# romanoshiliarhopoulos/Backgammon-Engine

Hardware: NVIDIA B200
Metric: selfplay_plies_per_sec (higher is better)
Workload: dtype f32

## Files before the change

### backgammon-engine_b200/csrc/bgx_kernels.cuh

```cuda
#pragma once
#include "bgx_device.cuh"
#include "bgx_ply.cuh"

namespace bgx {

constexpr int kGameWarps = 16;
constexpr int kGameThreads = kGameWarps * 32;
struct WarpSeat {
    long long slot;
    unsigned long long gid;
    int ply, step, status, player;
    int carry;
    int dice_base;
};

template <int kWarps, int kSets>
constexpr int ply_smem()
{
    return kFixedBytes + kWarps * (int)sizeof(PlyScratch<kSets>) + (int)sizeof(StealShared<kWarps>) + kWarps * (int)sizeof(WarpSeat) + 16;
}

template <int W, int S>
struct PlyConfig {
    static constexpr int kWarps = W, kSets = S, kSmem = ply_smem<W, S>();
// ... 7 lines not shown
    {
        int rc = 0;
        ((rc = rc ? rc : f(C{})), ...);
        return rc;
    }
    template <typename F>
    static void dispatch(int warps, F &&f) { ((warps == C::kWarps ? f(C{}) : void()), ...); }
};
using PlyConfigs = PlyConfigList<PlyConfig<16, 109>, PlyConfig<20, 86>, PlyConfig<24, 72>, PlyConfig<32, 53>>;
constexpr int kEvalSmem = kFixedBytes + 16;

constexpr int kUniqSlots = 4096;
constexpr int kUniqWords = 8;
constexpr size_t kUniqBytesPerWarp = (size_t)kUniqSlots * kUniqWords * 4;

__global__ void k_build_table(const float *__restrict__ flat, float *__restrict__ Wt)
{
    const int idx = blockIdx.x * blockDim.x + threadIdx.x;
    if (idx >= kTableFloats) return;
    const int f = idx / kHidden, j = idx % kHidden;
    Wt[idx] = flat[j * kFeatures + f];
}

__global__ void k_fixed_scale(const float *__restrict__ flat, float *__restrict__ aux)
{
    __shared__ float red[kHidden / 32];
    const int j = threadIdx.x;
    const float *w = flat + j * kFeatures;
    float bound = fabsf(flat[kTableFloats + j]);
    for (int i = 0; i < 24; i++) {
        float worst = 0.f;
        for (int c = 0; c < 2; c++) {
            const float *u = w + 8 * i + 4 * c;
            const float s1 = u[0], s2 = s1 + u[1], s3 = s2 + u[2];
            worst = fmaxf(worst, fmaxf(fabsf(s1), fabsf(s2)));
            worst = fmaxf(worst, fabsf(s3) + 6.f * fabsf(u[3]));
        }
        bound += worst;
    }
    bound += fmaxf(fabsf(w[192]), fabsf(w[193])) + 7.5f * (fabsf(w[194]) + fabsf(w[195])) + fabsf(w[196]) + fabsf(w[197]);
    float w2sum = fabsf(flat[kTableFloats + kHidden + j]);
    for (int o = 16; o > 0; o >>= 1) {
        bound = fmaxf(bound, __shfl_xor_sync(kFull, bound, o));
        w2sum += __shfl_xor_sync(kFull, w2sum, o);
    }
    __shared__ float red2[kHidden / 32];
    if ((j & 31) == 0) { red[j >> 5] = bound; red2[j >> 5] = w2sum; }
    __syncthreads();
    if (j == 0) {
        for (int k = 1; k < kHidden / 32; k++) { bound = fmaxf(bound, red[k]); w2sum += red2[k]; }
        int e = 30 - (ilogbf(fmaxf(bound, 1e-30f)) + 1);
        e = e > 60 ? 60 : (e < -60 ? -60 : e);
        aux[0] = ldexpf(1.f, e);
        aux[1] = ldexpf(1.f, -e);
        aux[2] = bound;
        int ey = 30 - (ilogbf(fmaxf(w2sum, 1e-30f)) + 1);
        ey = ey > 40 ? 40 : (ey < -60 ? -60 : ey);
        aux[3] = ldexpf(1.f, ey);
    }
}

__global__ void k_build_fixed(const float *__restrict__ flat, const float *__restrict__ aux, int32_t *__restrict__ Ti)
{
    const int idx = blockIdx.x * blockDim.x + threadIdx.x;
    if (idx >= kFixedInts) return;
    const int f = idx / kHidden, j = idx % kHidden;
    const float S = aux[0];
    if (f < kFeatures) {
        const float w = flat[j * kFeatures + f];
        const bool half = (f < 192 && (f & 3) == 3) || f == 194 || f == 195;
        Ti[idx] = f >= 196 ? __float_as_int(w) : __float2int_rn(w * (half ? 0.5f * S : S));
    } else if (f < kRowB1) {
        const int p = (f - kFeatures) / 15, k = (f - kFeatures) % 15;
        const float w = flat[j * kFeatures + 196 + p];
        Ti[idx] = __float2int_rn(w * (kOffFeature[k + 1] * S)) - __float2int_rn(w * (kOffFeature[k] * S));
    } else if (f == kRowB1) {
        Ti[idx] = __float2int_rn(flat[kTableFloats + j] * S);
    } else if (f == kRowW2) {
        Ti[idx] = __float_as_int(flat[kTableFloats + kHidden + j]);
    } else if (f == kRowConst) {
        const float c[4] = {S, -1.4426950408889634f * aux[1], flat[kTableFloats + 2 * kHidden], aux[3]};
        Ti[idx] = __float_as_int(c[j & 3]);
    } else {
        Ti[idx] = j < 32 ? (int32_t)ply_hash_multiplier(j) : 0;
    }
}

__device__ __forceinline__ long long claim(unsigned long long *counter, int lane)
{
    unsigned long long i = 0;
    if (lane == 0) i = atomicAdd(counter, 1ull);
    return (long long)__shfl_sync(kFull, i, 0);
}

__device__ __forceinline__ int load_record_byte(const int8_t *rec, int lane) { return (int)rec[lane]; }

struct SummaryLeaf {
    uint32_t *table;
    uint32_t gen;
    int lane;
    int n_seq = 0, n_unique = 0;
    bool overflow = false;
    uint64_t digest = 0;

    __device__ __forceinline__ void operator()(int v, uint64_t moves, int)
    {
        uint32_t k[5];
        key_planes(v, k);
        n_seq++;
        digest = digest * kDigestMul + leaf_hash(k, moves);
        if (overflow) return;
        const uint32_t k4g = k[4] | (gen << 24);
        const int w = lane & 7;
        const uint32_t mine = w == 0 ? k[0] : w == 1 ? k[1] : w == 2 ? k[2] : w == 3 ? k[3] : k4g;
        uint32_t bucket = hash_planes(k) & (kUniqSlots / 4 - 1);
        for (int probe = 0; probe < kUniqSlots / 4; probe++) {
            uint32_t *line = table + (size_t)bucket * 32;
            const uint32_t got = line[lane];
            const uint32_t same = __ballot_sync(kFull, w >= 5 || got == mine);
            const uint32_t stale = __ballot_sync(kFull, w == 4 && (got >> 24) != gen);
            for (int s = 0; s < 4; s++) {
                if (((same >> (8 * s)) & 0xFFu) == 0xFFu) return;
                if ((stale >> (8 * s + 4)) & 1u) {
                    if ((lane >> 3) == s && w < 5) line[lane] = mine;
                    __syncwarp();
                    n_unique++;
                    return;
                }
            }
            bucket = (bucket + 1) & (kUniqSlots / 4 - 1);
        }
        overflow = true;
    }
};

__global__ void __launch_bounds__(kGameThreads, 1)
k_enumerate_summary(const int8_t *__restrict__ queries, long long n, int32_t *__restrict__ n_seq,
                    int32_t *__restrict__ n_unique, unsigned long long *__restrict__ digest,
                    uint32_t *__restrict__ tables, uint32_t *__restrict__ gens, unsigned long long *counter)
{
    const int lane = threadIdx.x & 31;
    const int gwarp = blockIdx.x * (blockDim.x >> 5) + warp_index();
    uint32_t *table = tables + (size_t)gwarp * (kUniqBytesPerWarp / 4);
    uint32_t gen = gens[gwarp];
    for (;;) {
        const long long q = claim(counter, lane);
        if (q >= n) break;
        const int b = load_record_byte(queries + q * 32, lane);
        const int root = lane < 28 ? b : 0;
        const int player = __shfl_sync(kFull, b, 28), d1 = __shfl_sync(kFull, b, 29), d2 = __shfl_sync(kFull, b, 30);
        gen = (gen + 1) & 0xFFu;
        if (gen == 0) {
            for (int i = lane; i < kUniqSlots * kUniqWords; i += 32) table[i] = 0;
            gen = 1;
            __syncwarp();
        }
        SummaryLeaf leaf;
        leaf.table = table; leaf.gen = gen; leaf.lane = lane;
        walk_turn(root, lane, player, d1, d2, leaf);
        if (lane == 0) {
            n_seq[q] = leaf.n_seq;
            n_unique[q] = leaf.overflow ? -1 : leaf.n_unique;
            digest[q] = leaf.digest;
        }
        __syncwarp();
    }
    if (lane == 0) gens[gwarp] = gen;
// ... 308 lines not shown
    for (int j = warp; j < kOrderCtaQueries; j += 8) {
        const long long q = q0 + j;
        if (q >= n) break;
        const int b = load_record_byte(queries + q * 32, lane);
        const int player = __shfl_sync(kFull, b, 28) ? 1 : 0, d1 = __shfl_sync(kFull, b, 29), d2 = __shfl_sync(kFull, b, 30);
        const int k = order_bucket(lane < 28 ? b : 0, lane, player, d1, d2);
        if (lane == 0) { key[j] = (uint8_t)k; atomicAdd(&hist[k], 1u); }
    }
    __syncthreads();
    if (threadIdx.x < kOrderBuckets) {
        const uint32_t c = hist[threadIdx.x];
        base[threadIdx.x] = c ? atomicAdd(&totals[threadIdx.x], c) : 0u;
        hist[threadIdx.x] = 0;
    }
    __syncthreads();
    if (threadIdx.x < kOrderCtaQueries && q0 + threadIdx.x < n) {
        const int k = key[threadIdx.x];
        region[(size_t)k * n + base[k] + atomicAdd(&hist[k], 1u)] = (int32_t)(q0 + threadIdx.x);
    }
}

struct AdvanceOut {
    int8_t *next;
    int8_t *winner;
    const int32_t *ply_of;
    const long long *game_id;
    uint32_t seed_lo, seed_hi;
    int32_t *next_region;
    uint32_t *next_totals;
    long long id_stride;
    int first_mover;
    int32_t *ply_out;
    long long *gid_out;
};

__device__ __forceinline__ void store_advanced(const AdvanceOut &a, long long q, long long n, int v, int lane, int player)
{
    const int off1 = __shfl_sync(kFull, v, 26), off2 = __shfl_sync(kFull, v, 27);
    const int win = off1 == 15 ? 0 : (off2 == 15 ? 1 : -1);
    unsigned long long g = a.game_id ? (unsigned long long)a.game_id[q] : (unsigned long long)q;
    int ply = a.ply_of ? a.ply_of[q] : 0;
    int mover = win < 0 ? player ^ 1 : player, status = win + 1;
    if (a.id_stride > 0) {
        ply++;
        if (win >= 0) {
            g += (unsigned long long)a.id_stride;
            ply = 0;
            v = start_value(lane);
            mover = first_mover_of(a.seed_lo, a.seed_hi, g, a.first_mover);
            status = kRunning;
        }
    }
    const Philox r = philox4x32_10(a.seed_lo, a.seed_hi, (uint32_t)ply, (uint32_t)g, (uint32_t)(g >> 32), 0u);
    const int d1 = die_of(r.x[0]), d2 = die_of(r.x[1]);
    const int tail = lane == 28 ? mover : lane == 29 ? d1 : lane == 30 ? d2 : status;
    a.next[q * 32 + lane] = (int8_t)(lane < 28 ? v : tail);
    if (lane == 0) {
        if (a.winner) a.winner[q] = (int8_t)win;
        if (a.ply_out) a.ply_out[q] = ply;
        if (a.gid_out) a.gid_out[q] = (long long)g;
    }
    if (a.next_region) {
        const int b = status == kRunning ? order_bucket(lane < 28 ? v : 0, lane, mover, d1, d2) : 6;
        if (lane == 0) a.next_region[(size_t)b * n + atomicAdd(&a.next_totals[b], 1u)] = (int32_t)q;
    }
}

struct SelectTune {
    unsigned long long urgent_from;
    int urgent_min, giant_min;
};

template <int kWarps, int kSets, bool kExplore>
__global__ void __launch_bounds__(kWarps * 32, 1)
k_select(const int8_t *__restrict__ queries, long long n, float epsilon, uint32_t seed_lo, uint32_t seed_hi,
         SelectOut out, const int32_t *__restrict__ Ti, const float *__restrict__ flat,
         unsigned long long *counter, StealResult *__restrict__ steal, SelectTune tune,
         const int32_t *__restrict__ region, const uint32_t *__restrict__ totals, AdvanceOut adv)
{
    extern __shared__ __align__(128) unsigned char smem[];
    const PlySmem<kWarps, kSets> sm(smem);
    const int lane = threadIdx.x & 31, warp = warp_index();
    PlyCache<kSets> cache;
    cache.reset(sm.scratch[warp].cache, reinterpret_cast<const int4 *>(sm.table), lane);
    sm.init_share();
    stage_table(sm.table, Ti, sm.bar, kFixedBytes);
    PlyEvaluator ev;
    ev.T4 = reinterpret_cast<const int4 *>(sm.table);
    StealResult *cta_results = steal + (size_t)blockIdx.x * kWarps * kStealMaxResults;
    const ShareCtx mine = {&sm.share->slot[warp], cta_results + warp * kStealMaxResults, &sm.share->urgent, 1u << warp,
                           counter, tune.urgent_from, tune.urgent_min, tune.giant_min};
    bool helping = false, first = true;
    const long long first_wave = (long long)gridDim.x * kWarps;
    uint32_t bucket_end = 0;
    if (region) {
        bucket_end = lane < kOrderBuckets ? totals[kOrderBuckets - 1 - lane] : 0u;
#pragma unroll
        for (int o = 1; o < kOrderBuckets; o <<= 1) {
            const uint32_t up = __shfl_up_sync(kFull, bucket_end, o);
            if (lane >= o) bucket_end += up;
        }
    }
    for (;;) {
        int root = 0, player = 0, d1 = 0, d2 = 0, vw = 0;
        uint32_t only = 0, u = 0;
        long long q = 0;
        bool explore = false;
        if (helping || *(volatile uint32_t *)&sm.share->urgent != 0) {
            bool done;
            only = take_child<kWarps>(sm.share, lane, vw, root, player, d1, done, !helping);
            d2 = d1;
            if (helping && only == 0) {
                if (done) break;
                continue;
            }
        }
        if (only == 0) {
            q = first ? (long long)warp * gridDim.x + blockIdx.x : first_wave + claim(counter, lane);
            first = false;
            if (q >= n) {
                helping = true;
                if (lane == 0) atomicSub(&sm.share->active, 1);
                __syncwarp();
                continue;
            }
            if (region) {
                const int r = __popc(__ballot_sync(kFull, lane < kOrderBuckets && (uint32_t)q >= bucket_end));
                const uint32_t before = __shfl_sync(kFull, bucket_end, r > 0 ? r - 1 : 0);
                q = region[(size_t)(kOrderBuckets - 1 - r) * n + ((uint32_t)q - (r > 0 ? before : 0u))];
            }
            const int b = load_record_byte(queries + q * 32, lane);
            root = lane < 28 ? b : 0;
            player = __shfl_sync(kFull, b, 28) ? 1 : 0; d1 = __shfl_sync(kFull, b, 29); d2 = __shfl_sync(kFull, b, 30);
            if (kExplore && epsilon > 0.f) {
                const Philox r = philox4x32_10(seed_lo, seed_hi, 0u, (uint32_t)q, (uint32_t)((unsigned long long)q >> 32), 2u);
                explore = (float)r.x[0] * 2.3283064365386963e-10f < epsilon;
                u = r.x[1];
            }
        }
        d1 = __shfl_sync(kFull, d1, 0); d2 = __shfl_sync(kFull, d2, 0);
        player = __shfl_sync(kFull, player, 0); only = __shfl_sync(kFull, only, 0);
        const Choice c = choose_ply_fast<kSets, kExplore>(root, lane, player, d1, d2, ev, cache, explore, u, only ? only : kFull,
                                                          only ? nullptr : &mine);
        if (only) deliver_child<kWarps>(sm.share, cta_results, vw, only, c, lane);
        else {
            store_choice(out, q, c, lane, player);
            if (adv.next) store_advanced(adv, q, n, c.v, lane, player);
        }
        __syncwarp();
    }
}

__global__ void k_advance(const int8_t *chosen, int8_t *next, long long n, uint32_t seed_lo,
                          uint32_t seed_hi, int ply, const long long *__restrict__ game_id, int8_t *__restrict__ winner,
                          const int32_t *__restrict__ ply_of = nullptr)
{
    const long long warps = (long long)gridDim.x * (blockDim.x >> 5);
    const int lane = threadIdx.x & 31;
    for (long long q = (long long)blockIdx.x * (blockDim.x >> 5) + warp_index(); q < n; q += warps) {
        const int b = load_record_byte(chosen + q * 32, lane);
        const int off1 = __shfl_sync(kFull, b, 26), off2 = __shfl_sync(kFull, b, 27), mover = __shfl_sync(kFull, b, 28) ? 1 : 0;
        const int win = off1 == 15 ? 0 : (off2 == 15 ? 1 : -1);
        const unsigned long long g = game_id ? (unsigned long long)game_id[q] : (unsigned long long)q;
        const Philox r = philox4x32_10(seed_lo, seed_hi, (uint32_t)(ply_of ? ply_of[q] : ply), (uint32_t)g, (uint32_t)(g >> 32), 0u);
        const int tail = lane == 28 ? (win < 0 ? mover ^ 1 : mover) : lane == 29 ? die_of(r.x[0]) : lane == 30 ? die_of(r.x[1]) : win + 1;
        next[q * 32 + lane] = (int8_t)(lane < 28 ? b : tail);
        if (winner && lane == 0) winner[q] = (int8_t)win;
    }
}

struct SelfplayParams {
    int8_t *slots;
    int32_t *ply;
    long long *game_id;
    int8_t *traj_pre;
    int8_t *traj_chosen;
    long long n_slots, id_stride;
    uint32_t seed_lo, seed_hi;
    int first_mover, traj_cap;
    int n_plies;
    int round_mode;
    float epsilon;
    unsigned long long *counter;
    unsigned long long *stats;
    int4 *zstash;
};

template <int kWarps, int kSets, bool kExplore>
__global__ void __launch_bounds__(kWarps * 32, 1)
k_selfplay(SelfplayParams p, const int32_t *__restrict__ Ti, const float *__restrict__ flat, StealResult *__restrict__ steal)
{
    extern __shared__ __align__(128) unsigned char smem[];
    const PlySmem<kWarps, kSets> sm(smem);
    const int lane = threadIdx.x & 31, warp = warp_index();
    PlyCache<kSets> cache;
    cache.reset(sm.scratch[warp].cache, reinterpret_cast<const int4 *>(sm.table), lane);
    sm.init_share();
    stage_table(sm.table, Ti, sm.bar, kFixedBytes);
    PlyEvaluator ev;
    ev.T4 = reinterpret_cast<const int4 *>(sm.table);
    StealResult *cta_results = steal + (size_t)blockIdx.x * kWarps * kStealMaxResults;
    const ShareCtx mine = {&sm.share->slot[warp], cta_results + warp * kStealMaxResults, &sm.share->urgent, 1u << warp,
                           p.counter, (unsigned long long)(p.n_slots - p.n_slots / 4), 8, kGiantMinChildren};

    unsigned long long *cta_stats = sm.share->stats;
    const int budget = p.round_mode ? 0x7fffffff : p.n_plies;
    bool helping = false, seated = false;
    int v = 0, dice = 0;
    WarpSeat &S = sm.seat[warp];
    int4 *const zmine = p.zstash + ((size_t)blockIdx.x * kWarps + warp) * 32 + lane;
    for (;;) {
        int root = 0, mover = 0, d1 = 0, d2 = 0, vw = 0;
        uint32_t only = 0, u = 0;
        bool explore = false, rec_traj = false;
        if (helping || *(volatile uint32_t *)&sm.share->urgent != 0) {
            bool done;
            only = take_child<kWarps>(sm.share, lane, vw, root, mover, d1, done, !helping);
            d2 = d1;
            if (helping && only == 0) {
                if (done) break;
                continue;
            }
        }
        if (only == 0) {
            if (!seated) {
                const long long slot = claim(p.counter, lane);
                if (slot >= p.n_slots) {
                    helping = true;
                    if (lane == 0) atomicSub(&sm.share->active, 1);
                    __syncwarp();
                    continue;
                }
                const int b = load_record_byte(p.slots + slot * 32, lane);
                v = lane < 28 ? b : 0;
                const int status = __shfl_sync(kFull, b, 31);
                if (p.round_mode && status != kRunning) continue;
                const int mover0 = __shfl_sync(kFull, b, 28) ? 1 : 0;
                if (lane == 0) {
                    S.slot = slot;
                    S.player = mover0;
                    S.status = status;
                    S.ply = p.ply[slot];
                    S.gid = (unsigned long long)p.game_id[slot];
                    S.step = 0;
                    S.carry = 0;
                    S.dice_base = -1;
                }
                __syncwarp();
                seated = true;
            }
            const int ply = S.ply;
            if (p.round_mode && p.traj_cap > 0 && ply >= p.traj_cap) {
                if (lane == 0) S.status = kTruncated;
                __syncwarp();
                if (lane == 0) atomicAdd(cta_stats + 5, 1ull);
                seated = false;
            } else {
                const unsigned long long gid = S.gid;
                int ahead = ply - S.dice_base;
                if (S.dice_base < 0 || ahead < 0 || ahead >= 32) {
                    const Philox r = philox4x32_10(p.seed_lo, p.seed_hi, (uint32_t)(ply + lane), (uint32_t)gid, (uint32_t)(gid >> 32), 0u);
                    dice = die_of(r.x[0]) | (die_of(r.x[1]) << 4);
                    __syncwarp();
                    if (lane == 0) S.dice_base = ply;
                    __syncwarp();
                    ahead = 0;
                }
                const int rolled = __shfl_sync(kFull, dice, ahead);
                d1 = rolled & 15; d2 = rolled >> 4;
                mover = S.player;
                rec_traj = p.traj_pre != nullptr && ply < p.traj_cap && S.status == kRunning;
                if (rec_traj) {
                    int8_t *t = p.traj_pre + ((size_t)S.slot * p.traj_cap + ply) * 32;
                    const int out = lane < 28 ? v : (lane == 28 ? mover : (lane == 29 ? d1 : (lane == 30 ? d2 : 0)));
                    t[lane] = (int8_t)out;
                }
                if (kExplore && p.epsilon > 0.f) {
                    const Philox e = philox4x32_10(p.seed_lo, p.seed_hi, (uint32_t)ply, (uint32_t)gid, (uint32_t)(gid >> 32), 2u);
                    explore = (float)e.x[0] * 2.3283064365386963e-10f < p.epsilon;
// ... 136 lines not shown
```

### backgammon-engine_b200/csrc/bgx_ply.cuh

```cuda
#pragma once
#include <climits>

#include "bgx_device.cuh"

namespace bgx {

constexpr int kPlyEntryBytes = 32;

template <int kSets>
struct __align__(16) PlyScratch {
    uint8_t cache[kSets * 2 * kPlyEntryBytes];
};

__device__ __forceinline__ float fast_sigmoid(float z)
{
    float e, r;
    asm("ex2.approx.ftz.f32 %0, %1;" : "=f"(e) : "f"(z * -1.4426950408889634f));
    asm("rcp.approx.ftz.f32 %0, %1;" : "=f"(r) : "f"(1.0f + e));
    return r;
}

__device__ __forceinline__ float sigmoid_exp2(float a)
{
    float e, r;
    asm("ex2.approx.ftz.f32 %0, %1;" : "=f"(e) : "f"(a));
    asm("rcp.approx.ftz.f32 %0, %1;" : "=f"(r) : "f"(1.0f + e));
    return r;
}

__device__ __constant__ float kOffFeature[17] = {
    (float)(0 / 15.0), (float)(1 / 15.0), (float)(2 / 15.0), (float)(3 / 15.0), (float)(4 / 15.0), (float)(5 / 15.0),
    (float)(6 / 15.0), (float)(7 / 15.0), (float)(8 / 15.0), (float)(9 / 15.0), (float)(10 / 15.0), (float)(11 / 15.0),
    (float)(12 / 15.0), (float)(13 / 15.0), (float)(14 / 15.0), (float)(15 / 15.0), (float)(16 / 15.0)};

struct PlyEvaluator {
    const int4 *T4;

    __device__ __forceinline__ static void add(int4 &z, const int4 &t) { z.x += t.x; z.y += t.y; z.z += t.z; z.w += t.w; }
    __device__ __forceinline__ static void sub(int4 &z, const int4 &t) { z.x -= t.x; z.y -= t.y; z.z -= t.z; z.w -= t.w; }
    __device__ __forceinline__ static void addn(int4 &z, int n, const int4 &t) { z.x += n * t.x; z.y += n * t.y; z.z += n * t.z; z.w += n * t.w; }
    __device__ __forceinline__ int4 off_term(int k, int player, int lane) const
    {
        const int4 w = T4[(196 + player) * 32 + lane];
        const float f = kOffFeature[k] * __int_as_float(T4[kRowConst * 32 + lane].x);
        return make_int4(__float2int_rn(__int_as_float(w.x) * f), __float2int_rn(__int_as_float(w.y) * f),
                         __float2int_rn(__int_as_float(w.z) * f), __float2int_rn(__int_as_float(w.w) * f));
    }
    __device__ __forceinline__ int4 preactivation(int v, int lane, int turn) const
    {
        const int n = v < 0 ? -v : v;
        const int packed = (8 * lane + (v > 0 ? 0 : 4)) | (n << 8);
        uint32_t occ = __ballot_sync(kFull, lane < 24 && v != 0);
        int4 z = T4[kRowB1 * 32 + lane];
        while (occ) {
            const int i = lowest_bit(occ);
            occ &= occ - 1;
            const int p = __shfl_sync(kFull, packed, i);
            const int base = p & 0xFF, cnt = p >> 8;
            const int4 *row = T4 + base * 32 + lane;
            add(z, row[0]);
            if (cnt >= 2) add(z, row[32]);
            if (cnt >= 3) add(z, row[64]);
            if (cnt >= 4) addn(z, cnt - 3, row[96]);
        }
        add(z, T4[(192 + turn) * 32 + lane]);
        const int bar1 = __shfl_sync(kFull, v, 24), bar2 = __shfl_sync(kFull, v, 25);
        const int off1 = __shfl_sync(kFull, v, 26), off2 = __shfl_sync(kFull, v, 27);
        if (bar1) addn(z, bar1, T4[194 * 32 + lane]);
        if (bar2) addn(z, bar2, T4[195 * 32 + lane]);
        if (off1) add(z, off_term(off1, 0, lane));
        if (off2) add(z, off_term(off2, 1, lane));
        return z;
    }
    __device__ __forceinline__ int output_sum(const int4 &zi, int lane) const
    {
        const int4 wi = T4[kRowW2 * 32 + lane], ci = T4[kRowConst * 32];
        const float c = __int_as_float(ci.y), Y = __int_as_float(ci.w);
        const float y = __int_as_float(wi.x) * sigmoid_exp2((float)zi.x * c) + __int_as_float(wi.y) * sigmoid_exp2((float)zi.y * c) +
                        __int_as_float(wi.z) * sigmoid_exp2((float)zi.z * c) + __int_as_float(wi.w) * sigmoid_exp2((float)zi.w * c);
        return __reduce_add_sync(kFull, __float2int_rn(y * Y));
    }
    __device__ __forceinline__ float value_of(int total) const
    {
        const int4 ci = T4[kRowConst * 32];
        const float inv_y = __int_as_float(0x7F000000 - ci.w);
        return fast_sigmoid(fmaf((float)total, inv_y, __int_as_float(ci.z)));
    }
    __device__ __forceinline__ float finish(const int4 &zi, int lane) const { return value_of(output_sum(zi, lane)); }
};

template <int kSets>
struct PlyCache {
    uint8_t *col;
    uint32_t meta;
    const uint32_t *kmul;

    struct Probe {
        uint32_t off;
        uint32_t m0, m1;
        uint32_t h, got0, got1;
        __device__ __forceinline__ bool hit() const { return m0 == kFull || m1 == kFull; }
    };

    __device__ __forceinline__ void clear(int lane) const
    {
        uint32_t *w = reinterpret_cast<uint32_t *>(col - lane);
        for (int i = lane; i < kSets * 2 * kPlyEntryBytes / 4; i += 32) w[i] = 0;
    }
    __device__ __forceinline__ void reset(uint8_t *p, const int4 *T4, int lane)
    {
        col = p + lane;
        meta = 0;
        kmul = reinterpret_cast<const uint32_t *>(T4 + kRowLane * 32) + lane;
        clear(lane);
    }
    __device__ __forceinline__ void next_ply(int lane)
    {
        uint32_t gen = (__shfl_sync(kFull, meta, 29) + 1) & 0xFFu;
        if (gen == 0) {
            clear(lane);
            gen = 1;
            __syncwarp();
        }
        meta = lane == 29 ? gen : 0u;
    }
    template <int kTag>
    __device__ __forceinline__ uint32_t byte_of(int v, int lane) const
    {
        uint32_t b = ((uint32_t)v & 0xFFu) | meta;
        if (kTag != 0) b |= lane == 28 ? (uint32_t)kTag : 0u;
        return b;
    }
    template <int kTag>
    __device__ __forceinline__ Probe probe(int v, int lane) const
    {
        Probe p;
        const uint32_t h = __reduce_add_sync(kFull, (uint32_t)v * *kmul) + (uint32_t)kTag * 0x9E3779B1u;
        p.h = h;
        p.off = __umulhi(h, (uint32_t)kSets) * (2 * kPlyEntryBytes);
        const uint8_t *e = col + p.off;
        p.got0 = e[0];
        p.got1 = e[kPlyEntryBytes];
        const uint32_t mine = byte_of<kTag>(v, lane);
        p.m0 = __ballot_sync(kFull, p.got0 == mine);
        p.m1 = __ballot_sync(kFull, p.got1 == mine);
        if (kTag != 0) { p.m0 |= 0x40000000u; p.m1 |= 0x40000000u; }
        return p;
    }
    template <int kTag>
    __device__ __forceinline__ void write(const Probe &p, int v, int count, int lane) const
    {
        const uint32_t way = (p.m0 >> 29) & (~(p.m1 >> 29) | (p.h >> 20)) & 1u;
        uint32_t mine = byte_of<kTag>(v, lane);
        if (kTag != 0) mine |= lane == 30 ? (uint32_t)count : 0u;
        col[p.off + way * kPlyEntryBytes] = (uint8_t)mine;
    }
    template <int kTag>
    __device__ __forceinline__ int lookup(int v, int lane) const
    {
        const Probe p = probe<kTag>(v, lane);
        const int cnt = (int)__shfl_sync(kFull, p.m0 == kFull ? p.got0 : p.got1, 30);
        return p.hit() ? cnt : -1;
    }
    template <int kTag>
    __device__ __forceinline__ void store(int v, int count, int lane) const
    {
        if (count > 255) return;
        const Probe p = probe<kTag>(v, lane);
        if (!p.hit()) write<kTag>(p, v, count, lane);
    }
};

constexpr int kSeenBefore = INT_MIN;
template <int kSets>
__device__ __noinline__ int score_early_leaf(uint8_t *col, uint32_t meta, const uint32_t *kmul, const int4 *T4, int v, int lane, int player)
{
    PlyCache<kSets> cache;
    cache.col = col; cache.meta = meta; cache.kmul = kmul;
    const typename PlyCache<kSets>::Probe pr = cache.template probe<0>(v, lane);
    if (pr.hit()) return kSeenBefore;
    cache.template write<0>(pr, v, 0, lane);
    PlyEvaluator e;
    e.T4 = T4;
    return e.output_sum(e.preactivation(v, lane, player), lane);
}

template <int kSets>
struct PlyWalk : Mover {
    const PlyEvaluator &ev;
    const PlyCache<kSets> &cache;
    const int4 *Tme;
    int dieA, dieB;
    uint32_t root_only;
    uint32_t twin_root;
    bool nd;
    int4 zroot;
    int4 *zstash;
    bool z_ok;
    float best_key;
    int best_sum;
    int best_v;
    uint32_t best_path;
    int n_seq, n_scored, n_visited;

    __device__ __forceinline__ PlyWalk(const PlyEvaluator &e, const PlyCache<kSets> &c, int ln, int pl)
        : Mover(ln, pl), ev(e), cache(c)
    {
        Tme = e.T4 + ln + (pl ? 4 * 32 : 0);
        root_only = kFull;
        twin_root = 0;
        nd = false;
        best_key = __int_as_float(0xff800000);
        best_sum = INT_MIN;
        best_v = 0; best_path = 0;
        n_seq = n_scored = n_visited = 0;
        zstash = nullptr; z_ok = false;
    }

    __device__ __forceinline__ uint32_t move_word(int sval, int dval, int src, int dst) const
    {
        const int n = sval < 0 ? -sval : sval;
        const int row_src = src >= 24 ? 194 - 3 * player : 8 * src + (n < 4 ? n : 4) - 1;
        const int k = (dval < 0 ? -dval : dval) + 1;
        const bool hit = dst < 24 && dval * unit_of_points() == -1;
        int row_dst = dst >= 24 ? kFeatures + 11 * player + dval : 8 * dst + (k < 4 ? k : 4) - 1;
        if (hit) row_dst = 8 * dst;
        return (uint32_t)dst | (hit ? 32u : 0u) | ((uint32_t)row_src & 0xFFu) << 16 | (uint32_t)row_dst << 24;
    }
    __device__ __forceinline__ uint32_t node_moves(int v, int die) const
    {
        const int d = lane + die * unit_of_points();
        int dl = (unsigned)d > 23u ? 26 + player : d;
        if (lane >= 24) dl = player ? 24 - die : die - 1;
        return move_word(v, __shfl_sync(kFull, v, dl), lane, dl);
    }
    __device__ __forceinline__ int origin_lane(int o) const { return o == (player ? 25 : 0) ? 24 + player : o - 1; }

    __device__ __forceinline__ int apply_word(int v, int sl, uint32_t mv) const
    {
        const int dl = (int)(mv & 31u);
        const uint32_t hit = (mv >> 5) & 1u;
        int t = lane == dl ? unit << hit : 0;
        t -= lane == sl ? unit : 0;
        t += (lane == 25 - player ? 1 : 0) & (int)hit;
        return v + t;
    }

    __device__ __forceinline__ int4 child_z(const int4 &zpar, uint32_t mv) const
    {
        int4 z = zpar;
        PlyEvaluator::sub(z, Tme[((mv >> 16) & 0xFFu) * 32]);
        if (mv & 32u) {
            const int dst = (int)(mv & 31u);
            PlyEvaluator::sub(z, Tme[(8 * dst + 4 - 8 * player) * 32]);
            PlyEvaluator::add(z, Tme[(195 - 5 * player) * 32]);
        }
        PlyEvaluator::add(z, Tme[(mv >> 24) * 32]);
        return z;
    }

    template <int D>
    __device__ __forceinline__ void leaf(int v, const int4 &zpar, uint32_t mv, uint32_t path)
    {
        n_seq++;
        const typename PlyCache<kSets>::Probe pr = cache.template probe<0>(v, lane);
        if (pr.hit()) return;
        cache.template write<0>(pr, v, 0, lane);
        const int4 z = D == 0 ? zroot : child_z(zpar, mv);
        const int total = ev.output_sum(z, lane);
        n_scored++;
        const int sum = player ? -total : total;
        if (sum > best_sum) {
            const float val = ev.value_of(total);
            const float key = player ? -val : val;
            if (key > best_key) {
                best_key = key; best_sum = sum; best_v = v; best_path = path | ((uint32_t)D << 20);
                if (zstash) { *zstash = z; z_ok = true; }
            }
        }
    }

    __device__ __forceinline__ void early_leaf(int v, uint32_t path_and_len)
    {
        n_seq++;
        const int total = __shfl_sync(kFull, score_early_leaf<kSets>(cache.col, cache.meta, cache.kmul, ev.T4, v, lane, player), 0);
        if (total == kSeenBefore) return;
        n_scored++;
        const int sum = player ? -total : total;
        if (sum > best_sum) {
            const float val = ev.value_of(total);
            const float key = player ? -val : val;
            if (key > best_key) { best_key = key; best_sum = sum; best_v = v; best_path = path_and_len; z_ok = false; }
        }
    }

    template <int D>
    __device__ __forceinline__ void visit(int v, const int4 &zpar, uint32_t mv, bool left, uint32_t path, uint32_t legal_par = 0)
    {
        constexpr int kMax = 4;
        uint32_t legal = 0;
        if constexpr (D < kMax) {
            if (D == 1 && nd) legal = 1u;
            else legal = legal_here(v, (D & 1) ? dieB : dieA);
            if (D == 0) legal &= root_only;
        }
        uint32_t twins = 0;
        if constexpr (D == kMax - 1) {
            const int die = (D & 1) ? dieB : dieA;
            const int o = (int)((path >> (5 * (D - 1))) & 31u);
            twins = legal & (nd ? twin_root : legal_par & ((1u << o) - 1u));
            twins &= player ? ~((2u << die) - 1u) : (1u << (25 - die)) - 1u;
            if (left) twins = 0;
        }
        if (legal == 0) {
            if constexpr (D == kMax) leaf<D>(v, zpar, mv, path);
            else if (!(D == 2 && nd)) early_leaf(v, path | ((uint32_t)D << 20));
            return;
        }
        if constexpr (D < kMax) {
            if constexpr (D >= 2) {
                if (!nd) {
                    const int below = cache.template lookup<D>(v, lane);
                    if (below >= 0) { n_seq += below; return; }
                }
            }
            const int entered = n_seq;
            const uint32_t legal_all = legal;
            n_seq += __popc(twins);
            legal &= ~twins;
            if (D == kMax - 1 && legal == 0) {
                if constexpr (D >= 2) { if (!nd) cache.template store<D>(v, n_seq - entered, lane); }
                return;
            }
            int4 z = zroot;
            if (D != 0 && !(D <= 2 && nd)) z = child_z(zpar, mv);
            const int die = (D & 1) ? dieB : dieA;
            const uint32_t moves = (D == 1 && nd) ? 0u : node_moves(v, die);
            do {
                const int oc = lowest_bit(legal);
                legal &= legal - 1;
                int child = v;
                uint32_t mc = 0;
                bool off = false;
                if (!(D == 1 && nd)) {
                    const int sc = origin_lane(oc);
                    mc = __shfl_sync(kFull, moves, sc);
                    child = apply_word(v, sc, mc);
                    if (D + 1 == kMax - 1) off = (unsigned)(oc + die * unit_of_points() - 1) > 23u;
                    n_visited++;
                }
                visit<D + 1>(child, z, mc, off, path | ((uint32_t)oc << (5 * D)), legal_all);
            } while (legal);
            if constexpr (D >= 2) { if (!nd) cache.template store<D>(v, n_seq - entered, lane); }
        }
    }
};

constexpr int kStealMinChildren = 4;
constexpr int kGiantMinChildren = 10;
constexpr int kStealMaxResults = 16;

struct StealSlot {
    uint32_t legal0;
    int32_t pending;
    uint32_t nres;
    uint32_t meta;
    int8_t root[32];
};

struct __align__(16) StealResult {
    float value;
    int32_t any, n_seq, n_scored, n_visited, origin;
    unsigned long long moves;
    int8_t v[32];
};

template <int kWarps>
struct StealShared {
    StealSlot slot[kWarps];
    int32_t active;
    uint32_t urgent;
    int32_t pad[2];
    unsigned long long stats[8];
};

struct ShareCtx {
    StealSlot *slot;
    StealResult *results;
    uint32_t *urgent;
    uint32_t my_bit;
    const unsigned long long *queue;
    unsigned long long urgent_from;
    int urgent_min;
    int giant_min;
};

__device__ __forceinline__ Choice finish_choice(const uint32_t best_path, float best_key, int best_v, int n_seq, int n_scored,
                                                int n_visited, int root, int player, int d1, int d2, uint32_t best_pass)
{
    Choice best;
    best.any = n_seq > 0;
    best.v = best.any ? best_v : root;
    best.value = best.any ? (player ? -best_key : best_key) : __int_as_float(0x7fc00000);
    best.n_seq = n_seq; best.n_scored = n_scored; best.n_visited = n_visited;
    uint64_t mv = 0;
    if (best.any) {
        const int len = (int)(best_path >> 20);
        mv = (uint64_t)len << 40;
        for (int j = 0; j < len; j++) {
            const int o = (int)((best_path >> (5 * j)) & 31u);
            const int die = ((j & 1) != (int)best_pass) ? d2 : d1;
            mv |= pack_move(o, destination(player, o, die), j);
        }
    }
    best.moves = mv;
    best.z_ok = false;
    return best;
}

template <int kSets>
__device__ __forceinline__ Choice greedy_ply(int root, int lane, int player, int d1, int d2, const PlyEvaluator &ev,
                                             PlyCache<kSets> &cache, uint32_t root_only = kFull, const ShareCtx *share = nullptr,
                                             int4 *zstash = nullptr, bool carry = false)
{
    StealSlot *slot = share ? share->slot : nullptr;
    StealResult *results = share ? share->results : nullptr;
    cache.next_ply(lane);
    PlyWalk<kSets> w(ev, cache, lane, player);
    w.root_only = root_only;
    if (carry) {
        int4 z = *zstash;
        PlyEvaluator::sub(z, ev.T4[(193 - player) * 32 + lane]);
        PlyEvaluator::add(z, ev.T4[(192 + player) * 32 + lane]);
        w.zroot = z;
    } else {
        w.zroot = ev.preactivation(root, lane, player);
    }
    w.zstash = zstash;
    uint32_t best_pass = 0;
    bool shared = false;
    const bool dbl = d1 == d2;
    uint32_t legal = 0;
    float key1 = 0.f;
    int pass = 0;
    w.dieA = d1; w.dieB = d2;
    w.nd = !dbl;
    if (dbl) {
        legal = w.legal_here(root, d1) & root_only;
        if (legal == 0) {
            w.early_leaf(root, 0u);
        } else {
            shared = slot != nullptr && __popc(legal) >= kStealMinChildren;
            if (shared) {
                slot->root[lane] = (int8_t)root;
                if (lane == 0) { slot->meta = (uint32_t)player | ((uint32_t)d1 << 8); slot->nres = 0; }
                __threadfence_block();
                __syncwarp();
                if (lane == 0) {
                    atomicExch(&slot->legal0, legal);
                    const int kids = __popc(legal);
                    if (kids >= share->giant_min ||
                        (kids >= share->urgent_min && *(volatile const unsigned long long *)share->queue >= share->urgent_from))
                        atomicOr(share->urgent, share->my_bit);
                }
                __syncwarp();
            }
        }
    }
    const uint32_t root_moves = dbl ? w.node_moves(root, d1) : 0u;
    for (;;) {
        int child = root, oc = 0;
        uint32_t mroot = 0;
        if (dbl) {
            uint32_t bit = 0;
            if (shared) {
                for (;;) {
                    const uint32_t old = *(volatile uint32_t *)&slot->legal0;
                    if (old == 0) break;
                    const uint32_t low = old & (0u - old);
                    uint32_t was = 0;
                    if (lane == 0) was = atomicAnd(&slot->legal0, ~low);
                    was = __shfl_sync(kFull, was, 0);
                    if (was & low) { bit = low; break; }
                }
            } else {
                bit = legal & (0u - legal);
                legal &= legal - 1;
            }
            if (bit == 0) break;
            oc = lowest_bit(bit);
            const int sc = w.origin_lane(oc);
            mroot = __shfl_sync(kFull, root_moves, sc);
            child = w.apply_word(root, sc, mroot);
            w.n_visited++;
        } else {
            if (pass == 2) break;
            w.dieA = pass ? d2 : d1;
            w.dieB = pass ? d1 : d2;
            if (pass) { key1 = w.best_key; w.twin_root = w.legal_here(root, d1); }
            pass++;
        }
        w.template visit<1>(child, w.zroot, mroot, false, (uint32_t)oc);
    }
    if (dbl) {
        if (shared && lane == 0) atomicAnd(share->urgent, ~share->my_bit);
    } else {
        best_pass = w.best_key > key1 ? 1u : 0u;
        w.best_path = ((w.best_path & 0xFFFFFu) >> 10) | (((w.best_path >> 20) - 2u) << 20);
    }
    Choice best = finish_choice(w.best_path, w.best_key, w.best_v, w.n_seq, w.n_scored, w.n_visited, root, player, d1, d2, best_pass);
    best.z_ok = best.any && w.z_ok;
    if (shared) {
        while (*(volatile int32_t *)&slot->pending != 0) __nanosleep(64);
        __threadfence_block();
        const int n = (int)*(volatile uint32_t *)&slot->nres;
        int best_origin = best.any ? (int)(best.moves & 31u) : 99;
        for (int i = 0; i < n; i++) {
            const StealResult *r = results + i;
            const int any = __ldcg(&r->any);
            best.n_seq += __ldcg(&r->n_seq);
            best.n_scored += __ldcg(&r->n_scored);
            best.n_visited += __ldcg(&r->n_visited);
            if (!any) continue;
            const float val = __ldcg(&r->value);
            const int org = __ldcg(&r->origin);
            const bool better = !best.any || (player ? val < best.value : val > best.value) || (val == best.value && org < best_origin);
            if (better) {
                best.any = true; best.value = val; best_origin = org; best.z_ok = false;
                best.moves = __ldcg(&r->moves);
                best.v = (int)__ldcg(reinterpret_cast<const signed char *>(r->v) + lane);
            }
        }
    }
    return best;
}

template <int kWarps>
__device__ __forceinline__ uint32_t take_child(StealShared<kWarps> *sh, int lane, int &vw, int &root, int &player, int &die, bool &done,
                                               bool urgent_only = false)
{
    done = false;
    const uint32_t avail = lane < kWarps ? *(volatile uint32_t *)&sh->slot[lane].legal0 : 0u;
    uint32_t m = __ballot_sync(kFull, avail != 0);
    if (urgent_only) {
        m &= *(volatile uint32_t *)&sh->urgent;
        if (m == 0) return 0u;
    } else if (m == 0) {
        done = __shfl_sync(kFull, *(volatile int32_t *)&sh->active, 0) <= 0;
        if (!done) __nanosleep(200);
        return 0u;
    }
    vw = lowest_bit(m);
    StealSlot *vs = &sh->slot[vw];
    uint32_t bit = 0;
    if (lane == 0) {
        const uint32_t old = *(volatile uint32_t *)&vs->legal0;
        if (old) {
            const uint32_t high = 1u << highest_bit(old);
            atomicAdd(&vs->pending, 1);
            if (atomicCAS(&vs->legal0, old, old & ~high) == old) bit = high;
            else atomicSub(&vs->pending, 1);
        }
    }
    bit = __shfl_sync(kFull, bit, 0);
    if (bit == 0) return 0u;
    __threadfence_block();
    const int b = (int)*(volatile int8_t *)&vs->root[lane];
    const uint32_t meta = *(volatile uint32_t *)&vs->meta;
    root = lane < 28 ? b : 0;
    player = (int)(meta & 1u);
    die = (int)(meta >> 8);
    return bit;
}

template <int kWarps>
__device__ __forceinline__ void deliver_child(StealShared<kWarps> *sh, StealResult *cta_results, int vw, uint32_t bit, const Choice &c, int lane)
{
    StealSlot *vs = &sh->slot[vw];
    uint32_t idx = 0;
    if (lane == 0) idx = atomicAdd(&vs->nres, 1u);
    idx = __shfl_sync(kFull, idx, 0);
    StealResult *r = cta_results + vw * kStealMaxResults + idx;
    r->v[lane] = (int8_t)c.v;
    if (lane == 0) {
        r->value = c.value; r->any = c.any ? 1 : 0; r->n_seq = c.n_seq; r->n_scored = c.n_scored;
        r->n_visited = c.n_visited; r->origin = lowest_bit(bit); r->moves = c.moves;
    }
    __threadfence_block();
    __syncwarp();
    if (lane == 0) atomicSub(&vs->pending, 1);
    __syncwarp();
}

template <int kSets, bool kExplore>
__device__ __forceinline__ Choice choose_ply_fast(int root, int lane, int player, int d1, int d2, const PlyEvaluator &ev,
                                                  PlyCache<kSets> &cache, bool explore, uint32_t u,
                                                  uint32_t root_only = kFull, const ShareCtx *share = nullptr,
                                                  int4 *zstash = nullptr, bool carry = false)
{
    if (kExplore && explore) {
        CountLeaf cnt;
        walk_turn(root, lane, player, d1, d2, cnt);
        Choice c;
        c.v = root; c.moves = 0; c.value = __int_as_float(0x7fc00000); c.n_seq = cnt.n; c.n_scored = 0; c.n_visited = 0; c.any = cnt.n > 0;
        c.z_ok = false;
        if (cnt.n > 0) {
            PickLeaf pick((int)mulhi32(u, (uint32_t)cnt.n));
            walk_turn(root, lane, player, d1, d2, pick);
            c.v = pick.v;
            c.moves = pick.moves;
        }
        return c;
    }
    return greedy_ply<kSets>(root, lane, player, d1, d2, ev, cache, root_only, share, zstash, carry);
}

}
```

### backgammon-engine_b200/csrc/bgx_rollout.cuh

```cuda
#pragma once
#include "bgx_kernels.cuh"

namespace bgx {

constexpr int kRolloutStream = 4;

struct RolloutParams {
    const int8_t *positions;
    long long n_items;
    int trials, cap;
    int stratify;
    uint32_t seed_lo, seed_hi;
    float *value;
    int8_t *outcome;
    int32_t *plies;
    unsigned long long *counter;
    int4 *zstash;
};

__device__ __forceinline__ int outcome_class(int v, int lane, int winner)
{
    const int loser_off = __shfl_sync(kFull, v, 27 - winner);
    const int loser_bar = __shfl_sync(kFull, v, 25 - winner);
    const bool in_home = winner == 0 ? (lane >= 18 && lane < 24 && v < 0) : (lane < 6 && v > 0);
    const bool back = loser_bar != 0 || __ballot_sync(kFull, in_home) != 0;
    const int cls = loser_off != 0 ? 1 : (back ? 3 : 2);
    return winner == 0 ? cls : 3 + cls;
}

template <int kWarps, int kSets>
__global__ void __launch_bounds__(kWarps * 32, 1)
k_rollout(RolloutParams p, const int32_t *__restrict__ Ti, StealResult *__restrict__ steal)
{
    extern __shared__ __align__(128) unsigned char smem[];
    const PlySmem<kWarps, kSets> sm(smem);
    const int lane = threadIdx.x & 31, warp = warp_index();
    PlyCache<kSets> cache;
    cache.reset(sm.scratch[warp].cache, reinterpret_cast<const int4 *>(sm.table), lane);
    sm.init_share();
    stage_table(sm.table, Ti, sm.bar, kFixedBytes);
    PlyEvaluator ev;
    ev.T4 = reinterpret_cast<const int4 *>(sm.table);
    StealResult *cta_results = steal + (size_t)blockIdx.x * kWarps * kStealMaxResults;
    const ShareCtx mine = {&sm.share->slot[warp], cta_results + warp * kStealMaxResults, &sm.share->urgent, 1u << warp,
                           p.counter, (unsigned long long)(p.n_items - p.n_items / 4), 8, kGiantMinChildren};
    bool helping = false, seated = false;
    int v = 0, dice = 0;
    WarpSeat &S = sm.seat[warp];
    int4 *const zmine = p.zstash + ((size_t)blockIdx.x * kWarps + warp) * 32 + lane;
    for (;;) {
        int root = 0, mover = 0, d1 = 0, d2 = 0, vw = 0;
        uint32_t only = 0;
        if (helping || *(volatile uint32_t *)&sm.share->urgent != 0) {
            bool done;
            only = take_child<kWarps>(sm.share, lane, vw, root, mover, d1, done, !helping);
            d2 = d1;
            if (helping && only == 0) {
                if (done) break;
                continue;
            }
        }
        if (only == 0) {
            if (!seated) {
                const long long i = claim(p.counter, lane);
                if (i >= p.n_items) {
                    helping = true;
                    if (lane == 0) atomicSub(&sm.share->active, 1);
                    __syncwarp();
                    continue;
                }
                const long long pos = i / p.trials, t = i - pos * p.trials;
                const int b = load_record_byte(p.positions + pos * 32, lane);
                v = lane < 28 ? b : 0;
                const int off1 = __shfl_sync(kFull, v, 26), off2 = __shfl_sync(kFull, v, 27);
                if (off1 == 15 || off2 == 15) {
                    const int winner = off1 == 15 ? 0 : 1;
                    const int cls = outcome_class(v, lane, winner);
                    if (lane == 0) { p.value[i] = winner == 0 ? 1.f : 0.f; p.outcome[i] = (int8_t)cls; p.plies[i] = 0; }
                    __syncwarp();
                    continue;
                }
                const int mover0 = __shfl_sync(kFull, b, 28) ? 1 : 0;
                if (lane == 0) {
                    S.slot = i;
                    S.gid = (unsigned long long)t;
                    S.player = mover0;
                    S.ply = 0;
                    S.carry = 0;
                    S.dice_base = -1;
                }
                __syncwarp();
                seated = true;
            }
            const int ply = S.ply;
            const unsigned long long t = S.gid;
            int ahead = ply - S.dice_base;
            if (S.dice_base < 0 || ahead >= 32) {
                const Philox r = philox4x32_10(p.seed_lo, p.seed_hi, (uint32_t)(ply + lane), (uint32_t)t, (uint32_t)(t >> 32),
                                               (uint32_t)kRolloutStream);
                dice = die_of(r.x[0]) | (die_of(r.x[1]) << 4);
                __syncwarp();
                if (lane == 0) S.dice_base = ply;
                __syncwarp();
                ahead = 0;
            }
            const int rolled = __shfl_sync(kFull, dice, ahead);
            d1 = rolled & 15; d2 = rolled >> 4;
            if (p.stratify && ply == 0) {
                const int r = (int)(t % 36u);
                d1 = 1 + r / 6; d2 = 1 + r % 6;
            }
            mover = S.player;
            root = v;
        }
        d1 = __shfl_sync(kFull, d1, 0); d2 = __shfl_sync(kFull, d2, 0);
        mover = __shfl_sync(kFull, mover, 0); only = __shfl_sync(kFull, only, 0);
        const Choice c = choose_ply_fast<kSets, false>(root, lane, mover, d1, d2, ev, cache, false, 0u, only ? only : kFull,
                                                       only ? nullptr : &mine, only ? nullptr : zmine,
                                                       only == 0 && S.carry != 0);
        if (only) {
            deliver_child<kWarps>(sm.share, cta_results, vw, only, c, lane);
// ... 58 lines not shown
```

Baseline: 143.1 million.

## Canonicalize player-1 move search into mirrored frame to drop per-lane direction arithmetic

```diff
diff --git a/backgammon-engine_b200/csrc/bgx_kernels.cuh b/backgammon-engine_b200/csrc/bgx_kernels.cuh
--- a/backgammon-engine_b200/csrc/bgx_kernels.cuh
+++ b/backgammon-engine_b200/csrc/bgx_kernels.cuh
@@ -113,7 +113,10 @@
         const float c[4] = {S, -1.4426950408889634f * aux[1], flat[kTableFloats + 2 * kHidden], aux[3]};
         Ti[idx] = __float_as_int(c[j & 3]);
     } else {
-        Ti[idx] = j < 32 ? (int32_t)ply_hash_multiplier(j) : 0;
+        const int l = j & 31;
+        const int src = l < 24 ? 23 - l : (l < 28 ? l ^ 1 : l);
+        Ti[idx] = j < 32 ? (int32_t)ply_hash_multiplier(j)
+                : j < 64 ? (int32_t)(l < 24 ? 0u - ply_hash_multiplier(src) : ply_hash_multiplier(src)) : 0;
     }
 }
 
@@ -588,7 +591,7 @@
     const PlySmem<kWarps, kSets> sm(smem);
     const int lane = threadIdx.x & 31, warp = warp_index();
     PlyCache<kSets> cache;
-    cache.reset(sm.scratch[warp].cache, reinterpret_cast<const int4 *>(sm.table), lane);
+    cache.reset(sm.scratch[warp].cache, lane);
     sm.init_share();
     stage_table(sm.table, Ti, sm.bar, kFixedBytes);
     PlyEvaluator ev;
@@ -700,7 +703,7 @@
     const PlySmem<kWarps, kSets> sm(smem);
     const int lane = threadIdx.x & 31, warp = warp_index();
     PlyCache<kSets> cache;
-    cache.reset(sm.scratch[warp].cache, reinterpret_cast<const int4 *>(sm.table), lane);
+    cache.reset(sm.scratch[warp].cache, lane);
     sm.init_share();
     stage_table(sm.table, Ti, sm.bar, kFixedBytes);
     PlyEvaluator ev;
diff --git a/backgammon-engine_b200/csrc/bgx_ply.cuh b/backgammon-engine_b200/csrc/bgx_ply.cuh
--- a/backgammon-engine_b200/csrc/bgx_ply.cuh
+++ b/backgammon-engine_b200/csrc/bgx_ply.cuh
@@ -93,7 +93,6 @@
 struct PlyCache {
     uint8_t *col;
     uint32_t meta;
-    const uint32_t *kmul;
 
     struct Probe {
         uint32_t off;
@@ -107,11 +106,10 @@
         uint32_t *w = reinterpret_cast<uint32_t *>(col - lane);
         for (int i = lane; i < kSets * 2 * kPlyEntryBytes / 4; i += 32) w[i] = 0;
     }
-    __device__ __forceinline__ void reset(uint8_t *p, const int4 *T4, int lane)
+    __device__ __forceinline__ void reset(uint8_t *p, int lane)
     {
         col = p + lane;
         meta = 0;
-        kmul = reinterpret_cast<const uint32_t *>(T4 + kRowLane * 32) + lane;
         clear(lane);
     }
     __device__ __forceinline__ void next_ply(int lane)
@@ -132,10 +130,10 @@
         return b;
     }
     template <int kTag>
-    __device__ __forceinline__ Probe probe(int v, int lane) const
+    __device__ __forceinline__ Probe probe(int v, uint32_t hv, int lane) const
     {
         Probe p;
-        const uint32_t h = __reduce_add_sync(kFull, (uint32_t)v * *kmul) + (uint32_t)kTag * 0x9E3779B1u;
+        const uint32_t h = hv + (uint32_t)kTag * 0x9E3779B1u;
         p.h = h;
         p.off = __umulhi(h, (uint32_t)kSets) * (2 * kPlyEntryBytes);
         const uint8_t *e = col + p.off;
@@ -156,40 +154,52 @@
         col[p.off + way * kPlyEntryBytes] = (uint8_t)mine;
     }
     template <int kTag>
-    __device__ __forceinline__ int lookup(int v, int lane) const
-    {
-        const Probe p = probe<kTag>(v, lane);
+    __device__ __forceinline__ int lookup(int v, uint32_t hv, int lane) const
+    {
+        const Probe p = probe<kTag>(v, hv, lane);
         const int cnt = (int)__shfl_sync(kFull, p.m0 == kFull ? p.got0 : p.got1, 30);
         return p.hit() ? cnt : -1;
     }
     template <int kTag>
-    __device__ __forceinline__ void store(int v, int count, int lane) const
+    __device__ __forceinline__ void store(int v, uint32_t hv, int count, int lane) const
     {
         if (count > 255) return;
-        const Probe p = probe<kTag>(v, lane);
+        const Probe p = probe<kTag>(v, hv, lane);
         if (!p.hit()) write<kTag>(p, v, count, lane);
     }
 };
+
+__device__ __forceinline__ int mirror(int v, int lane)
+{
+    const int m = __shfl_sync(kFull, v, lane < 24 ? 23 - lane : (lane < 28 ? lane ^ 1 : lane));
+    return lane < 24 ? -m : m;
+}
 
 constexpr int kSeenBefore = INT_MIN;
 template <int kSets>
-__device__ __noinline__ int score_early_leaf(uint8_t *col, uint32_t meta, const uint32_t *kmul, const int4 *T4, int v, int lane, int player)
+__device__ __noinline__ int score_early_leaf(uint8_t *col, uint32_t meta, uint32_t hv, const int4 *T4, int v, int lane, int player)
 {
     PlyCache<kSets> cache;
-    cache.col = col; cache.meta = meta; cache.kmul = kmul;
-    const typename PlyCache<kSets>::Probe pr = cache.template probe<0>(v, lane);
+    cache.col = col; cache.meta = meta;
+    const typename PlyCache<kSets>::Probe pr = cache.template probe<0>(v, hv, lane);
     if (pr.hit()) return kSeenBefore;
     cache.template write<0>(pr, v, 0, lane);
     PlyEvaluator e;
     e.T4 = T4;
-    return e.output_sum(e.preactivation(v, lane, player), lane);
+    const int va = mirror(v, lane);
+    return e.output_sum(e.preactivation(player ? va : v, lane, player), lane);
 }
 
 template <int kSets>
-struct PlyWalk : Mover {
+struct PlyWalk {
     const PlyEvaluator &ev;
     const PlyCache<kSets> &cache;
+    int lane, player;
+    int flip;
+    const uint32_t *K;
     const int4 *Tme;
+    int fbase, fstride;
+    int bar_me, bar_en;
     int dieA, dieB;
     uint32_t root_only;
     uint32_t twin_root;
@@ -204,9 +214,14 @@
     int n_seq, n_scored, n_visited;
 
     __device__ __forceinline__ PlyWalk(const PlyEvaluator &e, const PlyCache<kSets> &c, int ln, int pl)
-        : Mover(ln, pl), ev(e), cache(c)
-    {
-        Tme = e.T4 + ln + (pl ? 4 * 32 : 0);
+        : ev(e), cache(c), lane(ln), player(pl)
+    {
+        flip = pl ? 31 : 0;
+        K = reinterpret_cast<const uint32_t *>(e.T4 + kRowLane * 32) + 32 * pl;
+        Tme = e.T4 + ln;
+        fbase = pl ? 8 * 23 + 4 : 0;
+        fstride = pl ? -8 : 8;
+        bar_me = 194 + pl; bar_en = 195 - pl;
         root_only = kFull;
         twin_root = 0;
         nd = false;
@@ -217,32 +232,58 @@
         zstash = nullptr; z_ok = false;
     }
 
+    __device__ __forceinline__ uint32_t hash(int v) const { return __reduce_add_sync(kFull, (uint32_t)v * K[lane]); }
+
+    __device__ __forceinline__ uint32_t legal_here(int v, int die) const
+    {
+        const uint32_t own = __ballot_sync(kFull, v > 0);
+        const uint32_t wall = __ballot_sync(kFull, v < -1) & 0xFFFFFFu;
+        const uint32_t pts = own & 0xFFFFFFu;
+        uint32_t legal;
+        if ((own >> 24) & 1u) {
+            legal = ((wall >> (die - 1)) & 1u) ? 0u : 1u << 24;
+        } else {
+            legal = pts & ((~wall & 0xFFFFFFu) >> die);
+            if (pts != 0 && (pts & 0x3FFFFu) == 0) {
+                legal |= pts & (1u << (24 - die));
+                if (player == 0) {
+                    const int hi = highest_bit(pts);
+                    if (hi + die > 24) legal |= 1u << hi;
+                } else {
+                    const uint32_t any = __ballot_sync(kFull, v != 0) & 0xFE0000u;
+                    const int lo = lowest_bit(any);
+                    if (lo + die > 24 && ((pts >> lo) & 1u)) legal |= 1u << lo;
+                }
+            }
+        }
+        return flip ? __brev(legal) : legal;
+    }
+
     __device__ __forceinline__ uint32_t move_word(int sval, int dval, int src, int dst) const
     {
-        const int n = sval < 0 ? -sval : sval;
-        const int row_src = src >= 24 ? 194 - 3 * player : 8 * src + (n < 4 ? n : 4) - 1;
-        const int k = (dval < 0 ? -dval : dval) + 1;
-        const bool hit = dst < 24 && dval * unit_of_points() == -1;
-        int row_dst = dst >= 24 ? kFeatures + 11 * player + dval : 8 * dst + (k < 4 ? k : 4) - 1;
-        if (hit) row_dst = 8 * dst;
-        return (uint32_t)dst | (hit ? 32u : 0u) | ((uint32_t)row_src & 0xFFu) << 16 | (uint32_t)row_dst << 24;
+        const int row_src = src >= 24 ? bar_me : fbase + fstride * src + (sval < 4 ? sval : 4) - 1;
+        const bool hit = dst < 24 && dval == -1;
+        int row_dst = dst >= 24 ? kFeatures + 15 * player + dval : fbase + fstride * dst + (dval < 3 ? dval : 3);
+        if (hit) row_dst = fbase + fstride * dst;
+        const int row_blot = fbase + (fstride >> 1) + fstride * dst;
+        return (uint32_t)dst | (hit ? 32u : 0u) | ((uint32_t)row_blot & 0xFFu) << 8 | ((uint32_t)row_src & 0xFFu) << 16 |
+               (uint32_t)row_dst << 24;
     }
     __device__ __forceinline__ uint32_t node_moves(int v, int die) const
     {
-        const int d = lane + die * unit_of_points();
-        int dl = (unsigned)d > 23u ? 26 + player : d;
-        if (lane >= 24) dl = player ? 24 - die : die - 1;
+        int dl = lane + die;
+        if (dl > 23) dl = 26;
+        if (lane >= 24) dl = die - 1;
         return move_word(v, __shfl_sync(kFull, v, dl), lane, dl);
     }
-    __device__ __forceinline__ int origin_lane(int o) const { return o == (player ? 25 : 0) ? 24 + player : o - 1; }
 
     __device__ __forceinline__ int apply_word(int v, int sl, uint32_t mv) const
     {
         const int dl = (int)(mv & 31u);
-        const uint32_t hit = (mv >> 5) & 1u;
-        int t = lane == dl ? unit << hit : 0;
-        t -= lane == sl ? unit : 0;
-        t += (lane == 25 - player ? 1 : 0) & (int)hit;
+        const int hit = (int)((mv >> 5) & 1u);
+        int t = lane == dl ? 1 << hit : 0;
+        t -= lane == sl ? 1 : 0;
+        t += (lane == 25 ? 1 : 0) & hit;
         return v + t;
     }
 
@@ -251,9 +292,8 @@
         int4 z = zpar;
         PlyEvaluator::sub(z, Tme[((mv >> 16) & 0xFFu) * 32]);
         if (mv & 32u) {
-            const int dst = (int)(mv & 31u);
-            PlyEvaluator::sub(z, Tme[(8 * dst + 4 - 8 * player) * 32]);
-            PlyEvaluator::add(z, Tme[(195 - 5 * player) * 32]);
+            PlyEvaluator::sub(z, Tme[((mv >> 8) & 0xFFu) * 32]);
+            PlyEvaluator::add(z, Tme[bar_en * 32]);
         }
         PlyEvaluator::add(z, Tme[(mv >> 24) * 32]);
         return z;
@@ -263,7 +303,7 @@
     __device__ __forceinline__ void leaf(int v, const int4 &zpar, uint32_t mv, uint32_t path)
     {
         n_seq++;
-        const typename PlyCache<kSets>::Probe pr = cache.template probe<0>(v, lane);
+        const typename PlyCache<kSets>::Probe pr = cache.template probe<0>(v, hash(v), lane);
         if (pr.hit()) return;
         cache.template write<0>(pr, v, 0, lane);
         const int4 z = D == 0 ? zroot : child_z(zpar, mv);
@@ -283,7 +323,8 @@
     __device__ __forceinline__ void early_leaf(int v, uint32_t path_and_len)
     {
         n_seq++;
-        const int total = __shfl_sync(kFull, score_early_leaf<kSets>(cache.col, cache.meta, cache.kmul, ev.T4, v, lane, player), 0);
+        const uint32_t hv = hash(v);
+        const int total = __shfl_sync(kFull, score_early_leaf<kSets>(cache.col, cache.meta, hv, ev.T4, v, lane, player), 0);
         if (total == kSeenBefore) return;
         n_scored++;
         const int sum = player ? -total : total;
@@ -309,7 +350,8 @@
             const int die = (D & 1) ? dieB : dieA;
             const int o = (int)((path >> (5 * (D - 1))) & 31u);
             twins = legal & (nd ? twin_root : legal_par & ((1u << o) - 1u));
-            twins &= player ? ~((2u << die) - 1u) : (1u << (25 - die)) - 1u;
+            const uint32_t stay = (1u << 24) | ((1u << (24 - die)) - 1u);
+            twins &= flip ? __brev(stay) : stay;
             if (left) twins = 0;
         }
         if (legal == 0) {
@@ -318,9 +360,11 @@
             return;
         }
         if constexpr (D < kMax) {
+            uint32_t hv = 0;
             if constexpr (D >= 2) {
                 if (!nd) {
-                    const int below = cache.template lookup<D>(v, lane);
+                    hv = hash(v);
+                    const int below = cache.template lookup<D>(v, hv, lane);
                     if (below >= 0) { n_seq += below; return; }
                 }
             }
@@ -329,7 +373,7 @@
             n_seq += __popc(twins);
             legal &= ~twins;
             if (D == kMax - 1 && legal == 0) {
-                if constexpr (D >= 2) { if (!nd) cache.template store<D>(v, n_seq - entered, lane); }
+                if constexpr (D >= 2) { if (!nd) cache.template store<D>(v, hv, n_seq - entered, lane); }
                 return;
             }
             int4 z = zroot;
@@ -343,15 +387,15 @@
                 uint32_t mc = 0;
                 bool off = false;
                 if (!(D == 1 && nd)) {
-                    const int sc = origin_lane(oc);
+                    const int sc = oc ^ flip;
                     mc = __shfl_sync(kFull, moves, sc);
                     child = apply_word(v, sc, mc);
-                    if (D + 1 == kMax - 1) off = (unsigned)(oc + die * unit_of_points() - 1) > 23u;
+                    if (D + 1 == kMax - 1) off = sc < 24 && sc + die > 23;
                     n_visited++;
                 }
                 visit<D + 1>(child, z, mc, off, path | ((uint32_t)oc << (5 * D)), legal_all);
             } while (legal);
-            if constexpr (D >= 2) { if (!nd) cache.template store<D>(v, n_seq - entered, lane); }
+            if constexpr (D >= 2) { if (!nd) cache.template store<D>(v, hv, n_seq - entered, lane); }
         }
     }
 };
@@ -396,11 +440,12 @@
 };
 
 __device__ __forceinline__ Choice finish_choice(const uint32_t best_path, float best_key, int best_v, int n_seq, int n_scored,
-                                                int n_visited, int root, int player, int d1, int d2, uint32_t best_pass)
+                                                int n_visited, int root, int lane, int player, int d1, int d2, uint32_t best_pass)
 {
     Choice best;
     best.any = n_seq > 0;
-    best.v = best.any ? best_v : root;
+    const int va = mirror(best_v, lane);
+    best.v = best.any ? (player ? va : best_v) : root;
     best.value = best.any ? (player ? -best_key : best_key) : __int_as_float(0x7fc00000);
     best.n_seq = n_seq; best.n_scored = n_scored; best.n_visited = n_visited;
     uint64_t mv = 0;
@@ -408,7 +453,8 @@
         const int len = (int)(best_path >> 20);
         mv = (uint64_t)len << 40;
         for (int j = 0; j < len; j++) {
-            const int o = (int)((best_path >> (5 * j)) & 31u);
+            const int i = (int)((best_path >> (5 * j)) & 31u);
+            const int o = player ? (i == 7 ? 25 : i - 7) : (i == 24 ? 0 : i + 1);
             const int die = ((j & 1) != (int)best_pass) ? d2 : d1;
             mv |= pack_move(o, destination(player, o, die), j);
         }
@@ -440,15 +486,17 @@
     uint32_t best_pass = 0;
     bool shared = false;
     const bool dbl = d1 == d2;
+    const int va = mirror(root, lane);
+    const int froot = player ? va : root;
     uint32_t legal = 0;
     float key1 = 0.f;
     int pass = 0;
     w.dieA = d1; w.dieB = d2;
     w.nd = !dbl;
     if (dbl) {
-        legal = w.legal_here(root, d1) & root_only;
+        legal = w.legal_here(froot, d1) & root_only;
         if (legal == 0) {
-            w.early_leaf(root, 0u);
+            w.early_leaf(froot, 0u);
         } else {
             shared = slot != nullptr && __popc(legal) >= kStealMinChildren;
             if (shared) {
@@ -467,9 +515,9 @@
             }
         }
     }
-    const uint32_t root_moves = dbl ? w.node_moves(root, d1) : 0u;
+    const uint32_t root_moves = dbl ? w.node_moves(froot, d1) : 0u;
     for (;;) {
-        int child = root, oc = 0;
+        int child = froot, oc = 0;
         uint32_t mroot = 0;
         if (dbl) {
             uint32_t bit = 0;
@@ -489,15 +537,15 @@
             }
             if (bit == 0) break;
             oc = lowest_bit(bit);
-            const int sc = w.origin_lane(oc);
+            const int sc = oc ^ w.flip;
             mroot = __shfl_sync(kFull, root_moves, sc);
-            child = w.apply_word(root, sc, mroot);
+            child = w.apply_word(froot, sc, mroot);
             w.n_visited++;
         } else {
             if (pass == 2) break;
             w.dieA = pass ? d2 : d1;
             w.dieB = pass ? d1 : d2;
-            if (pass) { key1 = w.best_key; w.twin_root = w.legal_here(root, d1); }
+            if (pass) { key1 = w.best_key; w.twin_root = w.legal_here(froot, d1); }
             pass++;
         }
         w.template visit<1>(child, w.zroot, mroot, false, (uint32_t)oc);
@@ -508,7 +556,8 @@
         best_pass = w.best_key > key1 ? 1u : 0u;
         w.best_path = ((w.best_path & 0xFFFFFu) >> 10) | (((w.best_path >> 20) - 2u) << 20);
     }
-    Choice best = finish_choice(w.best_path, w.best_key, w.best_v, w.n_seq, w.n_scored, w.n_visited, root, player, d1, d2, best_pass);
+    Choice best = finish_choice(w.best_path, w.best_key, w.best_v, w.n_seq, w.n_scored, w.n_visited, root, lane, player, d1, d2,
+                                best_pass);
     best.z_ok = best.any && w.z_ok;
     if (shared) {
         while (*(volatile int32_t *)&slot->pending != 0) __nanosleep(64);
@@ -584,7 +633,7 @@
     r->v[lane] = (int8_t)c.v;
     if (lane == 0) {
         r->value = c.value; r->any = c.any ? 1 : 0; r->n_seq = c.n_seq; r->n_scored = c.n_scored;
-        r->n_visited = c.n_visited; r->origin = lowest_bit(bit); r->moves = c.moves;
+        r->n_visited = c.n_visited; r->origin = (int)(c.moves & 31u); r->moves = c.moves;
     }
     __threadfence_block();
     __syncwarp();
diff --git a/backgammon-engine_b200/csrc/bgx_rollout.cuh b/backgammon-engine_b200/csrc/bgx_rollout.cuh
--- a/backgammon-engine_b200/csrc/bgx_rollout.cuh
+++ b/backgammon-engine_b200/csrc/bgx_rollout.cuh
@@ -36,7 +36,7 @@
     const PlySmem<kWarps, kSets> sm(smem);
     const int lane = threadIdx.x & 31, warp = warp_index();
     PlyCache<kSets> cache;
-    cache.reset(sm.scratch[warp].cache, reinterpret_cast<const int4 *>(sm.table), lane);
+    cache.reset(sm.scratch[warp].cache, lane);
     sm.init_share();
     stage_table(sm.table, Ti, sm.bar, kFixedBytes);
     PlyEvaluator ev;
```

Measured after the change: 150.0 million (median of 6 runs). 4.8% higher.
